# yynil/RWKVTTS

Measured on AMD Instinct MI355X. Metric: audio-tokens/sec/GPU (train fwd+bwd) RWKV7-0.4B L=4096; 1->8 GPU scaling, higher is better.
Workload: dtype bf16; 1 GPU; RWKV7-0.4B Spark layout train step (fwd+bwd+AdamW), B=8/GPU L=4096, synthetic text+speech tokens, random init (BASELINE.json configs[1]); global_batch=8, seq_len=4096, parallelism=dp1, grad_allreduce=none

## Files before the change

rwkvtts_amd/backbone.py:

```python
from __future__ import annotations

import json
import math
import os
from dataclasses import asdict, dataclass, field
from typing import List, Optional

import torch
import torch.nn as nn
import torch.nn.functional as F

from . import fused, ops

HEAD_SIZE = 64


@dataclass
class RWKV7Config:
    hidden_size: int = 1024
    num_hidden_layers: int = 24
    head_dim: int = 64
    vocab_size: int = 8193
    decay_low_rank_dim: int = 64
    a_low_rank_dim: int = 64
# ... 269 lines not shown
            mus, w1s, acts, names = self.lora_branches()
            xr, xk, xv, hs = fused.mix_lora(x, mask, self.x_r, self.x_k, self.x_v, mus, w1s, acts)
            return self.forward_mixed((xr, None, xk, xv, None, None), x, mask, v_first, state, seq_start, resid, dict(zip(names, hs)))
        mixed = fused.token_shift_mix6(x, x_prev, self.x_r, self.x_w, self.x_k, self.x_v,
                                       self.x_a, self.x_g, mask, self._stacked_mix(x.dtype))
        return self.forward_mixed(mixed, x, mask, v_first, state, seq_start, resid)

    def lora_branches(self):
        loras = [self.w_lora, self.a_lora] + ([self.v_lora] if self.layer_idx != 0 else []) + [self.g_lora]
        mus = [self.x_w, self.x_a] + ([self.x_v] if self.layer_idx != 0 else []) + [self.x_g]
        names = ("w", "a") + (("v",) if self.layer_idx != 0 else ()) + ("g",)
        return mus, [l.lora[0].weight for l in loras], [l.activation for l in loras], names

    def mix_params(self):
        return (self.x_r, self.x_w, self.x_k, self.x_v, self.x_a, self.x_g)

    def forward_mixed(self, mixed, x, mask, v_first, state: Optional[LayerState] = None, seq_start=None, resid=None, hid=None,
                      diff_state=False, packed: Optional["_PackedState"] = None):
        xr, xw, xk, xv, xa, xg = mixed
        B, T, D = xr.shape
        H, N = self.num_heads, self.head_dim
        r = self.r_proj(xr)
        k = self.k_proj(xk)
        v_lo = None
        if hid is not None:
            v = self.v_proj(xv)
            w_pre = self.w_lora.lora[2](hid["w"])
            a_pre = self.a_lora.lora[2](hid["a"])
            g = self.g_lora.lora[2](hid["g"])
            v_pre = None if self.layer_idx == 0 else self.v_lora.lora[2](hid["v"])
        else:
            if (self.layer_idx != 0 and DUAL_LINEAR_XV and self.v_proj.bias is None
                    and fused.dual_linear_supported(xv, self.v_proj.weight, self.v_lora.lora[0].weight)):
                v, v_lo = fused.dual_linear(xv, self.v_proj.weight, self.v_lora.lora[0].weight)
            else:
                v = self.v_proj(xv)
            w_pre = self.w_lora(xw)
            a_pre = self.a_lora(xa)
            g = self.g_lora(xg)
            if self.layer_idx == 0:
                v_pre = None
            else:
                v_pre = self.v_lora.forward_from_hidden(v_lo) if v_lo is not None else self.v_lora(xv)
        if self.layer_idx == 0:
            if mask is not None:
                v = v * mask
            v_first = v
        if mask is not None:
            r = r * mask

        def core():
            y, vf_next = fused.tmix_core(r, w_pre, k, v, a_pre, g, v_pre, v_first, self.k_k, self.k_a, self.g_norm.weight,
                                         self.g_norm.bias, self.r_k, mask, H, self.g_norm.eps, self.layer_idx == 0, seq_start)
            if resid is not None and self.o_proj.bias is None:
                x1 = fused.linear_add(y, self.o_proj.weight, resid)
                if x1 is not None:
                    return (x1, True), (v_first if vf_next is None else vf_next)
            return self.o_proj(y), (v_first if vf_next is None else vf_next)

        if hid is not None:
            return core()
        if seq_start is not None or (state is None and torch.is_grad_enabled() and (r.requires_grad or w_pre.requires_grad)
                                     and FUSED_TMIX_CORE):
            return core()
        w, k2, v2, a_in, b_in = fused.tmix_prepare(w_pre, k, v, a_pre, v_pre, v_first, self.k_k, self.k_a, mask,
                                                   H, self.layer_idx == 0)
        if state is None:
            if torch.is_grad_enabled() and (r.requires_grad or w.requires_grad):
                y = ops.RUN_CUDA_RWKV7g(r, w, k2, v2, a_in, b_in)
            else:
                y = ops.wkv7_forward_nograd(r, w, k2, v2, a_in, b_in)
        elif packed is not None:
            w = packed.identity_w(w)
            y, hT = ops.wkv7_state_chunked_seq(state.att_kv, r.contiguous(), w, k2, v2, a_in, b_in, packed.seq_off, packed.nseq)
            _store(state, "att_kv", hT, diff_state)
            _store_last(state, "att_x_prev", x, packed, diff_state)
        elif diff_state:
            y, hT = ops.wkv7_state_chunked(state.att_kv, r.contiguous(), w, k2, v2, a_in, b_in)
            _store(state, "att_kv", hT, True)
            _store(state, "att_x_prev", _last_token(x, mask), True)
        else:
            y = ops.RWKV7_BATCH_OP(state.att_kv, r.contiguous(), w, k2, v2, a_in, b_in)
            _store(state, "att_x_prev", _last_token(x, mask), False)
        y = fused.tmix_post(y, r, k2, v2, g, self.g_norm.weight, self.g_norm.bias, self.r_k, H, self.g_norm.eps)
        return self.o_proj(y), v_first


class RWKV7FeedForward(nn.Module):

    def __init__(self, cfg: RWKV7Config, layer_idx: int):
        super().__init__()
        self.x_k = nn.Parameter(torch.zeros(cfg.hidden_size))
        self.key = Linear(cfg.hidden_size, cfg.intermediate_size, bias=False)
        self.value = Linear(cfg.intermediate_size, cfg.hidden_size, bias=False)

    def forward(self, x, mask, state: Optional[LayerState] = None, diff_state=False, packed: Optional["_PackedState"] = None):
        if packed is not None:
            kx = packed.carry((fused.token_shift_mix1(x, None, self.x_k, mask),), x, state.ffn_x_prev, (self.x_k,))[0]
            _store_last(state, "ffn_x_prev", x, packed, diff_state)
            return self.forward_mixed(kx)
        kx = fused.token_shift_mix1(x, None if state is None else state.ffn_x_prev, self.x_k, mask)
        if state is not None:
            _store(state, "ffn_x_prev", _last_token(x, mask), diff_state)
        return self.forward_mixed(kx)

    def forward_mixed(self, kx):
        if self.key.bias is None and self.value.bias is None:
            out = fused.channel_mix(kx, self.key.weight, self.value.weight)
            if out is not None:
                return out
        s = fused.key_relu_sq(kx, self.key.weight) if self.key.bias is None else None
        if s is None:
            h = self.key(kx)
            if self.value.bias is None:
                out = fused.relu_sq_value(h, self.value.weight)
                if out is not None:
                    return out
            s = fused.relu_sq(h)
        return self.value(s)


class RWKV7Block(nn.Module):
    def __init__(self, cfg: RWKV7Config, layer_idx: int):
        super().__init__()
        self.layer_idx = layer_idx
        D = cfg.hidden_size
        if layer_idx == 0:
            self.pre_norm = nn.LayerNorm(D, eps=cfg.norm_eps, bias=cfg.norm_bias)
        self.attn_norm = nn.LayerNorm(D, eps=cfg.norm_eps, bias=cfg.norm_bias)
        self.attn = RWKV7Attention(cfg, layer_idx)
        self.ffn_norm = nn.LayerNorm(D, eps=cfg.norm_eps, bias=cfg.norm_bias)
        self.ffn = RWKV7FeedForward(cfg, layer_idx)

    def forward(self, x, delta, mask, v_first, state: Optional[LayerState] = None, seq_start=None, diff_state=False,
                packed: Optional["_PackedState"] = None):
        if self.layer_idx == 0:
            if delta is not None:
                x = x + delta
                delta = None
            x = fused.layer_norm(x, self.pre_norm)
        if diff_state or packed is not None:
            if delta is None:
                h = fused.layer_norm(x, self.attn_norm)
            else:
                x, h = fused.add_layer_norm(x, delta, self.attn_norm)
            att, v_first = self.attn(h, mask, v_first, state, diff_state=diff_state, packed=packed)
            x, h = fused.add_layer_norm(x, att, self.ffn_norm)
            return x, self.ffn(h, mask, state, diff_state=diff_state, packed=packed), v_first
        one_pass = fused.add_ln_mix_supported(x, state)
        if one_pass and (FUSED_ADD_LN_MIX6 or FUSED_ADD_LN_MIX6_FWD):
            x, mixed = fused.add_layer_norm_mix(x, delta, self.attn_norm, mask, self.attn.mix_params(), fwd_only=not FUSED_ADD_LN_MIX6)
            att, v_first = self.attn.forward_mixed(mixed, None, mask, v_first, None, seq_start,
                                                   resid=x if FUSED_ADD_LN_MIX1 else None)
        elif (one_pass and FUSED_TMIX_CORE and fused.FUSED_ADD_LN_MIX_LORA_FWD and x.requires_grad
              and fused.mix_lora_supported(x, state, seq_start, self.attn.lora_branches()[1])):
            a = self.attn
            mus, w1s, acts, names = a.lora_branches()
            x, xr, xk, xv, hs = fused.add_layer_norm_mix_lora(x, delta, self.attn_norm, mask, a.x_r, a.x_k, a.x_v, mus, w1s, acts)
            att, v_first = a.forward_mixed((xr, None, xk, xv, None, None), None, mask, v_first, None, seq_start,
                                           x if FUSED_ADD_LN_MIX1 else None, dict(zip(names, hs)))
        else:
            if delta is None:
                h = fused.layer_norm(x, self.attn_norm)
            else:
                x, h = fused.add_layer_norm(x, delta, self.attn_norm)
            att, v_first = self.attn(h, mask, v_first, state, seq_start, resid=x if (one_pass and FUSED_ADD_LN_MIX1) else None)
        if one_pass and FUSED_ADD_LN_MIX1:
            if isinstance(att, tuple):
                x, (kx,) = fused.add_layer_norm_mix(att[0], None, self.ffn_norm, mask, (self.ffn.x_k,))
            else:
                x, (kx,) = fused.add_layer_norm_mix(x, att, self.ffn_norm, mask, (self.ffn.x_k,))
            return x, self.ffn.forward_mixed(kx), v_first
        x, h = fused.add_layer_norm(x, att, self.ffn_norm)
        return x, self.ffn(h, mask, state), v_first


class ModelOutput(dict):

    def __getattr__(self, k):
        try:
            return self[k]
        except KeyError as e:
            raise AttributeError(k) from e

    def __getitem__(self, k):
        if isinstance(k, int):
            return [v for v in self.values() if v is not None][k]
        return super().__getitem__(k)


class RWKV7Model(nn.Module):

    def __init__(self, cfg: RWKV7Config):
        super().__init__()
        self.config = cfg
        self.embeddings = nn.Embedding(cfg.vocab_size, cfg.hidden_size)
        self.layers = nn.ModuleList([RWKV7Block(cfg, i) for i in range(cfg.num_hidden_layers)])
        self.norm = nn.LayerNorm(cfg.hidden_size, eps=cfg.norm_eps, bias=cfg.norm_bias)
        self.gradient_checkpointing = False

    def forward(self, input_ids=None, attention_mask=None, inputs_embeds=None, past_key_values: Optional[Cache] = None,
                use_cache: Optional[bool] = None, cu_seqlens=None, attention_mask_all_ones: Optional[bool] = None, cache_rows=None,
                **kwargs):
        if (input_ids is None) == (inputs_embeds is None):
            raise ValueError("You must specify exactly one of input_ids or inputs_embeds")
        x = self.embeddings(input_ids) if inputs_embeds is None else inputs_embeds
        if cache_rows is not None:
            return self._forward_packed_rows(x, cu_seqlens, past_key_values, cache_rows)
        if cu_seqlens is not None:
            if past_key_values is not None and len(past_key_values) > 0:
                return self._forward_packed_state(x, cu_seqlens, past_key_values)
            return self._forward_packed(x, cu_seqlens)
        B, T, D = x.shape
        if not x.is_cuda:
            raise RuntimeError("RWKV7Model runs on the HIP device only (no CPU path); move the model and inputs to cuda")
        mask = None
        if attention_mask is not None:
            known = attention_mask_all_ones if attention_mask_all_ones is not None else getattr(attention_mask, "_rwkv7_all_ones", None)
            if known is not None and os.environ.get("RWKV7_CHECK_MASK_HINT") == "1":
                assert bool(attention_mask[:, -T:].all()) == bool(known), \
                    "attention mask hint (mark_all_ones / attention_mask_all_ones) contradicts the mask: marked before an in-place edit?"
            if not (known if known is not None else bool(attention_mask[:, -T:].all())):
                mask = attention_mask[:, -T:].to(x.dtype).unsqueeze(-1)
        if use_cache and past_key_values is None:
            past_key_values = Cache.zeros(self.config, B, x.device, x.dtype)
        stateful = past_key_values is not None and len(past_key_values) > 0
        diff_state = stateful and self._differentiable_state(past_key_values, x)
        pad = 0
        gran = ops.CHUNK_T if x.dtype == torch.bfloat16 else ops.CHUNK_LEN
        if not stateful and T % gran != 0:
            pad = gran - T % gran
            x = torch.cat([x.new_zeros(B, pad, D), x], 1)
            m = torch.ones(B, T, 1, dtype=x.dtype, device=x.device) if mask is None else mask
            mask = torch.cat([m.new_zeros(B, pad, 1), m], 1)
        x = self._run_layers(x, mask, past_key_values if stateful else None, diff_state=diff_state)
        if pad:
            x = x[:, pad:]
        if stateful:
            past_key_values.seen_tokens += T
        return ModelOutput(last_hidden_state=x, past_key_values=past_key_values if stateful else None)


    @staticmethod
    def _differentiable_state(cache: Cache, x) -> bool:
        if not torch.is_grad_enabled() or not cache.requires_grad:
            return False
        if x.dtype != torch.bfloat16:
            raise ValueError(f"training through a differentiable cache needs a bf16 model (the chunked backward is bf16 only), got {x.dtype}")
        return True

    def _run_layers(self, x, mask, cache: Optional[Cache], seq_start=None, diff_state=False, packed=None):
        v_first = delta = None
        for i, layer in enumerate(self.layers):
            if self.gradient_checkpointing and self.training and cache is None:
                x, delta, v_first = torch.utils.checkpoint.checkpoint(layer, x, delta, mask, v_first, None, seq_start,
                                                                      use_reentrant=False)
            else:
                x, delta, v_first = layer(x, delta, mask, v_first, None if cache is None else cache[i], seq_start,
                                          diff_state=diff_state, packed=packed)
        return fused.add_layer_norm(x, delta, self.norm)[1] if delta is not None else fused.layer_norm(x, self.norm)

    def _run_packed_aligned(self, x, cu_seqlens, t_al):
        dest, seq_off = _packed_layout(cu_seqlens, x.shape[1], t_al)
        rows = ops.RowMap(dest, t_al, x.device)
        out = self._run_layers(rows.to_aligned(x), rows.keep.to(x.dtype), None, seq_off.to(x.device, non_blocking=True))
        return ModelOutput(last_hidden_state=rows.to_packed(out), past_key_values=None)

    def _forward_packed_state(self, x, cu_seqlens, cache: Cache):
        n_rows = cache[0].att_kv.shape[0]
        cu = [int(c) for c in cu_seqlens.tolist()]
        N = len(cu) - 1
        if n_rows != N:
            raise ValueError(f"cu_seqlens holds {N} sequences but the cache has batch size {n_rows}: a packed row with a cache needs "
                             "one cache row per sequence")
        if x.dtype != torch.bfloat16:
            raise ValueError(f"cu_seqlens with a cache needs a bf16 model (the stateful packed scan is bf16 only), got {x.dtype}")
        if x.shape[0] != 1 or not x.is_cuda:
            raise ValueError("cu_seqlens expects a packed [1, total, D] row on the HIP device")
        total = x.shape[1]
        if any(b < a for a, b in zip(cu[:-1], cu[1:])) or cu[0] < 0 or cu[-1] > total:
            raise ValueError(f"cu_seqlens must be non-decreasing within [0, {total}], got {cu}")
        diff = self._differentiable_state(cache, x)
        lay = ops.packed_state_layout([b - a for a, b in zip(cu[:-1], cu[1:])], torch.is_grad_enabled(), align=_row_align)
        cache.seen_tokens += cu[-1] - cu[0]
        if lay.t_al == 0:
            return ModelOutput(last_hidden_state=x.new_zeros(x.shape), past_key_values=cache)
        dest = torch.full((total,), -1, dtype=torch.int32)
        dest[cu[0]:cu[-1]] = lay.dest
        rows = ops.RowMap(dest, lay.t_al, x.device)
        packed = _PackedState(lay, rows.keep, x.device)
        out = self._run_layers(rows.to_aligned(x), rows.keep.to(x.dtype), cache, diff_state=diff, packed=packed)
        return ModelOutput(last_hidden_state=rows.to_packed(out), past_key_values=cache)

    def _forward_packed_rows(self, x, cu_seqlens, cache: Cache, cache_rows):
        if cu_seqlens is None or cache is None or len(cache) == 0:
            raise ValueError("cache_rows needs cu_seqlens and past_key_values")
        if cache.requires_grad:
            raise ValueError("cache_rows updates the cache in place: a differentiable cache is not supported")
        rows = [int(r) for r in torch.as_tensor(cache_rows).reshape(-1).tolist()]
        n_rows, N = cache[0].att_kv.shape[0], cu_seqlens.numel() - 1
        if len(rows) != N:
            raise ValueError(f"cache_rows names {len(rows)} rows for {N} sequences")
        if len(set(rows)) != N or any(not 0 <= r < n_rows for r in rows):
            raise ValueError(f"cache_rows must be {N} distinct rows in [0, {n_rows}), got {rows}")
        idx = torch.tensor(rows, dtype=torch.int64).to(cache[0].att_kv.device, non_blocking=True)
        sub = Cache([LayerState(s.att_x_prev.index_select(0, idx), s.att_kv.index_select(0, idx), s.ffn_x_prev.index_select(0, idx))
                     for s in cache.states], cache.seen_tokens)
        out = self._forward_packed_state(x, cu_seqlens, sub)
# ... 114 lines not shown
```

rwkvtts_amd/csrc/ln_row.h:

```cpp
#pragma once
#include <type_traits>

#include "../../include/rwkv7_hip.h"
#include "wkv7_common.h"

namespace rwkv7 {

constexpr int kEwMaxThreads = 512;

typedef __bf16 pkbf2_t __attribute__((ext_vector_type(2)));
typedef float pkf2_t __attribute__((ext_vector_type(2)));
__device__ __forceinline__ uint32_t pk_bf16(float a, float b) {
    const pkf2_t v = {a, b};
    return __builtin_bit_cast(uint32_t, __builtin_convertvector(v, pkbf2_t));
}

template <typename T>
struct V8;
template <>
struct V8<bf16_t> {
    static __device__ __forceinline__ void ld(const bf16_t *p, float (&f)[8]) {
        const uint4 r = *reinterpret_cast<const uint4 *>(p);
        f[0] = __uint_as_float(r.x << 16); f[1] = __uint_as_float(r.x & 0xffff0000u);
        f[2] = __uint_as_float(r.y << 16); f[3] = __uint_as_float(r.y & 0xffff0000u);
        f[4] = __uint_as_float(r.z << 16); f[5] = __uint_as_float(r.z & 0xffff0000u);
        f[6] = __uint_as_float(r.w << 16); f[7] = __uint_as_float(r.w & 0xffff0000u);
    }
    static __device__ __forceinline__ void st(bf16_t *p, const float (&f)[8]) {
        uint4 r;
        r.x = pk_bf16(f[0], f[1]);
        r.y = pk_bf16(f[2], f[3]);
        r.z = pk_bf16(f[4], f[5]);
        r.w = pk_bf16(f[6], f[7]);
        *reinterpret_cast<uint4 *>(p) = r;
    }
    static __device__ __forceinline__ float ld1(const bf16_t *p) { return bf2f(p->x); }
};
template <>
struct V8<float> {
    static __device__ __forceinline__ void ld(const float *p, float (&f)[8]) {
        const float4 a = *reinterpret_cast<const float4 *>(p), b = *reinterpret_cast<const float4 *>(p + 4);
        f[0] = a.x; f[1] = a.y; f[2] = a.z; f[3] = a.w; f[4] = b.x; f[5] = b.y; f[6] = b.z; f[7] = b.w;
    }
    static __device__ __forceinline__ void st(float *p, const float (&f)[8]) {
        *reinterpret_cast<float4 *>(p) = make_float4(f[0], f[1], f[2], f[3]);
        *reinterpret_cast<float4 *>(p + 4) = make_float4(f[4], f[5], f[6], f[7]);
    }
    static __device__ __forceinline__ float ld1(const float *p) { return *p; }
};

template <typename T>
struct Raw8;
template <>
struct Raw8<bf16_t> {
    uint4 r;
    __device__ __forceinline__ void load(const bf16_t *p) { r = *reinterpret_cast<const uint4 *>(p); }
    __device__ __forceinline__ void get(float (&f)[8]) const {
        f[0] = __uint_as_float(r.x << 16); f[1] = __uint_as_float(r.x & 0xffff0000u);
        f[2] = __uint_as_float(r.y << 16); f[3] = __uint_as_float(r.y & 0xffff0000u);
        f[4] = __uint_as_float(r.z << 16); f[5] = __uint_as_float(r.z & 0xffff0000u);
        f[6] = __uint_as_float(r.w << 16); f[7] = __uint_as_float(r.w & 0xffff0000u);
    }
};
template <>
struct Raw8<float> {
    float4 a, b;
    __device__ __forceinline__ void load(const float *p) {
        a = *reinterpret_cast<const float4 *>(p);
        b = *reinterpret_cast<const float4 *>(p + 4);
    }
    __device__ __forceinline__ void get(float (&f)[8]) const {
        f[0] = a.x; f[1] = a.y; f[2] = a.z; f[3] = a.w; f[4] = b.x; f[5] = b.y; f[6] = b.z; f[7] = b.w;
    }
};

template <typename T>
__device__ __forceinline__ float round_to(float v);
template <>
__device__ __forceinline__ float round_to<bf16_t>(float v) { return __uint_as_float(pk_bf16(v, v) & 0xffff0000u); }
template <>
__device__ __forceinline__ float round_to<float>(float v) { return v; }

__device__ __forceinline__ float add_pinned(float a, float b) {
    float r;
    asm("v_add_f32 %0, %1, %2" : "=v"(r) : "v"(a), "v"(b));
    return r;
}
__device__ __forceinline__ float sum_slots(const float *red, int ngroups) {
    float t = 0.f;
    for (int i = 0; i < ngroups; i += 4) {
        const float4 v = *reinterpret_cast<const float4 *>(red + i);
        t = add_pinned(add_pinned(add_pinned(add_pinned(t, v.x), v.y), v.z), v.w);
    }
    return t;
}
template <int ROWS>
__device__ __forceinline__ void red_init(float (*red)[kEwMaxThreads / 8]) {
    for (int i = threadIdx.x; i < ROWS * (kEwMaxThreads / 8); i += blockDim.x) (&red[0][0])[i] = 0.f;
    __syncthreads();
}

__device__ __forceinline__ void block_sum2(float &a, float &b, float (*red)[kEwMaxThreads / 8], int ph, int ngroups) {
    a = sum8(a);
    b = sum8(b);
    if ((threadIdx.x & 7) == 0) {
        red[ph][threadIdx.x >> 3] = a;
        red[ph + 1][threadIdx.x >> 3] = b;
    }
    __syncthreads();
    const float ta = sum_slots(red[ph], ngroups), tb = sum_slots(red[ph + 1], ngroups);
    a = ta;
    b = tb;
}

template <typename T>
struct RowPre {
    Raw8<T> xv, bv;
    float m;
};

template <typename T>
__device__ __forceinline__ void add_ln_row(const RowPre<T> &f, long o, bool has_branch, bool has_mask, bool write, T *x_out, T *h_out,
                                           const float (&gm)[8], const float (&bt)[8], float inv_d, float eps, int ng,
                                           float (*red)[kEwMaxThreads / 8], int &ph, float &mu, float &rs, float (&hm)[8]) {
    float v[8];
    f.xv.get(v);
    if (has_branch) {
        float b[8];
        f.bv.get(b);
#pragma unroll
        for (int j = 0; j < 8; j++) v[j] = round_to<T>(v[j] + b[j]);
        if (write) V8<T>::st(x_out + o, v);
    }
    float s = 0.f, dummy = 0.f;
#pragma unroll
    for (int j = 0; j < 8; j++) s += v[j];
    block_sum2(s, dummy, red, ph, ng);
    ph ^= 2;
    mu = s * inv_d;
    float q = 0.f;
    dummy = 0.f;
#pragma unroll
    for (int j = 0; j < 8; j++) {
        v[j] -= mu;
        q = fmaf(v[j], v[j], q);
    }
    block_sum2(q, dummy, red, ph, ng);
    ph ^= 2;
    rs = rsqrtf(q * inv_d + eps);
    const float m = has_mask ? f.m : 1.f;
#pragma unroll
    for (int j = 0; j < 8; j++) hm[j] = round_to<T>(fmaf(v[j] * rs, gm[j], bt[j]));
    if (write && h_out) V8<T>::st(h_out + o, hm);
#pragma unroll
    for (int j = 0; j < 8; j++) hm[j] *= m;
}

inline bool row_width_ok(int D) { return D > 0 && D % 64 == 0 && D <= kEwMaxThreads * 8; }

template <typename... P, typename... A>
int launch_rows(void (*kernel)(P...), int nblocks, int D, hipStream_t st, A... args) {
    (void)hipGetLastError();
    hipLaunchKernelGGL(kernel, dim3(nblocks), dim3(D / 8), 0, st, args...);
    return (int)hipGetLastError();
}

template <int... NS, typename F>
int for_nmix(int nmix, F launch) {
    int rc = RWKV7_ESHAPE;
    (void)((nmix == NS && ((rc = launch(std::integral_constant<int, NS>{})), true)) || ...);
    return rc;
}

}
```

rwkvtts_amd/fused.py:

```python
import ctypes
import os

import torch

from . import _lib

_FWD_BLOCKS = 32768
_MIX_FWD_BLOCKS = 2048
_BWD_BLOCKS = 1024
_MIX_BWD_ROWS = 4
_MIX_BWD_BLOCKS = 1024


def _sfx(t):
    if not t.is_cuda:
        raise NotImplementedError("fused RWKV-7 stages run on the HIP device only (no CPU path)")
    if t.dtype == torch.bfloat16:
        return "bf16"
    if t.dtype == torch.float32:
        return "f32"
    raise TypeError(f"bf16 or fp32 expected, got {t.dtype}")


def _c(t):
# ... 52 lines not shown
    nmix = params.shape[0]
    gs = [torch.zeros_like(x) if g is None else _c(g) for g in gs]
    nb = _grid(B * T, _MIX_BWD_ROWS, _MIX_BWD_BLOCKS)
    dx = torch.empty_like(x)
    part = torch.empty(nb, nmix, D, dtype=torch.float32, device=x.device)
    _call("mix_bwd", x, B, T, D, nmix, _lib.ptr_array(gs), x, xp, mask, params, dx, part, nb, _MIX_BWD_ROWS)
    return dx, part, gs


class _Mix(torch.autograd.Function):

    @staticmethod
    def forward(ctx, x, x_prev, mask, params):
        x, params = _c(x), _c(params)
        xp = None if x_prev is None else _c(x_prev.to(x.dtype))
        out = _mix_fwd(x, xp, mask, params)
        ctx.save_for_backward(x, xp, mask, params)
        ctx.xp_dtype = None if x_prev is None else x_prev.dtype
        return tuple(out[i] for i in range(params.shape[0]))

    @staticmethod
    def backward(ctx, *gs):
        x, xp, mask, params = ctx.saved_tensors
        dx, part, gs = _mix_bwd(gs, x, xp, mask, params)
        dxp = None
        if ctx.needs_input_grad[1]:
            dxp = (params.float().unsqueeze(1) * torch.stack([g[:, 0, :] for g in gs]).float()).sum(0).to(ctx.xp_dtype)
        return dx, dxp, None, _colsum(part, params.dtype)


FUSED_MIX_LORA = os.environ.get("RWKV7_FUSED_MIX_LORA", "1") == "1"
FUSED_MIX_LORA_HITS = [0]
WGRAD_SLABS_WCAT = 32


def _wcat_grads(dx, dG, wcat, x):
    D = x.shape[-1]
    dG2 = _c(dG).view(-1, dG.shape[-1])
    dx.view(-1, D).addmm_(dG2, wcat)
    return wgrad_splitk(dG2, x.view(-1, D), slabs=WGRAD_SLABS_WCAT)


class _MixLora(torch.autograd.Function):

    @staticmethod
    def forward(ctx, x, mask, params, wcat):
        B, T, D = x.shape
        x, params, wcat = _c(x), _c(params), _c(wcat)
        out = _mix_fwd(x, None, mask, params)
        G = torch.mm(x.view(-1, D), wcat.t())
        ctx.save_for_backward(x, mask, params, wcat)
        FUSED_MIX_LORA_HITS[0] += 1
        return (*[out[i] for i in range(params.shape[0])], G.view(B, T, -1))

    @staticmethod
    def backward(ctx, *gs):
        x, mask, params, wcat = ctx.saved_tensors
        nmix = params.shape[0]
        dx, part, _ = _mix_bwd(gs[:nmix], x, None, mask, params)
        dwcat = None if gs[nmix] is None else _wcat_grads(dx, gs[nmix], wcat, x)
        return dx, None, _colsum(part, params.dtype), dwcat


def mix_lora_supported(x, state, seq_start, w1s=None, mask=None):
    if not (FUSED_MIX_LORA and state is None and (seq_start is None or mask is not None) and x.is_cuda and x.dtype == torch.bfloat16 and torch.is_grad_enabled()
            and x.requires_grad and x.dim() == 3 and x.shape[0] * x.shape[1] >= WGRAD_MIN_ROWS and x.shape[-1] % 8 == 0):
        return False
    if w1s is not None:
        w1s = w1s() if callable(w1s) else w1s
        return 0 < len(w1s) <= 4 and all(w.dtype == torch.bfloat16 and w.is_contiguous() and w.dim() == 2 and w.shape[0] % 8 == 0 for w in w1s)
    return True


def _wcat_fwd(w1s, mus):
    ranks = [w.shape[0] for w in w1s]
    D = w1s[0].shape[1]
    wcat = torch.empty(2 * sum(ranks), D, dtype=w1s[0].dtype, device=w1s[0].device)
    _lib.call("rwkv7_mix_lora_wcat_fwd_bf16", wcat, len(w1s), _ints(ranks), _lib.ptr_array(w1s), _lib.ptr_array(mus), D, wcat)
    return wcat


def _wcat_bwd(dwcat, w1s, mus):
    nb = len(w1s)
    D = w1s[0].shape[1]
    dw1 = [torch.empty_like(w) for w in w1s]
    dmu = [torch.empty(D, dtype=w1s[0].dtype, device=w1s[0].device) for _ in range(nb)]
    _lib.call("rwkv7_mix_lora_wcat_bwd_bf16", dwcat, nb, _ints([w.shape[0] for w in w1s]), _lib.ptr_array(w1s), _lib.ptr_array(mus), D,
              dwcat, _lib.ptr_array(dw1), _lib.ptr_array(dmu))
    return dw1, dmu


class _WcatBuild(torch.autograd.Function):

    @staticmethod
    def forward(ctx, nb, *ts):
        w1s, mus = [_c(t) for t in ts[:nb]], [_c(t) for t in ts[nb:]]
        ctx.save_for_backward(*w1s, *mus)
        ctx.nb = nb
        ctx.mu_shapes = [t.shape for t in ts[nb:]]
        return _wcat_fwd(w1s, mus)

    @staticmethod
    def backward(ctx, dwcat):
        ts = ctx.saved_tensors
        dw1, dmu = _wcat_bwd(_c(dwcat), ts[:ctx.nb], ts[ctx.nb:])
        return (None, *dw1, *[g.view(sh) for g, sh in zip(dmu, ctx.mu_shapes)])


_ACT_CODE = {None: 0, "tanh": 1, "sigmoid": 2}


def _combine_bwd(das, outs, mask, ranks, acts, shape):
    B, T = outs[0].shape[:2]
    das = [torch.zeros_like(o) if g is None else _c(g) for g, o in zip(das, outs)]
    dG = torch.empty(shape, dtype=outs[0].dtype, device=outs[0].device)
    _lib.call("rwkv7_mix_lora_combine_bwd_bf16", dG, len(ranks), _ints(ranks), _ints(acts), B * T, T, mask, _lib.ptr_array(outs),
              _lib.ptr_array(das), dG)
    return dG


class _CombineAct(torch.autograd.Function):

    @staticmethod
    def forward(ctx, G, mask, ranks, acts):
        B, T, R2 = G.shape
        G = _c(G)
        outs = [torch.empty(B, T, r, dtype=G.dtype, device=G.device) for r in ranks]
        _lib.call("rwkv7_mix_lora_combine_fwd_bf16", G, len(ranks), _ints(ranks), _ints(acts), B * T, T, G, mask, _lib.ptr_array(outs))
        ctx.save_for_backward(mask, *outs)
        ctx.ranks, ctx.acts, ctx.shape = ranks, acts, (B, T, R2)
        return tuple(outs)

    @staticmethod
    def backward(ctx, *das):
        mask, *outs = ctx.saved_tensors
        return _combine_bwd(das, outs, mask, ctx.ranks, ctx.acts, ctx.shape), None, None, None


LORA_DOWN_DIRECT = os.environ.get("RWKV7_LORA_DOWN_DIRECT", "1") == "1"
LORA_DOWN_DIRECT_HITS = [0]


def lora_down_direct_supported(x, w1s):
    B, T, D = x.shape
    ranks = [w.shape[0] for w in w1s]
    if not (LORA_DOWN_DIRECT and (B * T) % 128 == 0 and D % 128 == 0 and D <= 4096 and all(r % 32 == 0 for r in ranks)):
        return False
    tiles = [b for b, r in enumerate(ranks) for _ in range(r // 32)]
    ok = lambda h: 1 <= len(h) <= 5 and len(set(h)) <= 2
    lds = 2 * (3 * 129 * 72 + 2 * len(tiles) * 2048 + len(ranks) * D)
    return 2 <= len(tiles) <= 10 and lds <= 160 * 1024 and any(ok(tiles[:c]) and ok(tiles[c:]) for c in range(1, len(tiles)))


class _MixLoraDirect(torch.autograd.Function):

    @staticmethod
    def forward(ctx, x, mask, params, nb, acts, *ts):
        B, T, D = x.shape
        x, params = _c(x), _c(params)
        w1s, mus = [_c(t) for t in ts[:nb]], [_c(t.reshape(-1)) for t in ts[nb:]]
        out = _mix_fwd(x, None, mask, params)
        ranks = [w.shape[0] for w in w1s]
        cr = _ints(ranks)
        packed = torch.empty(sum(ranks), D, dtype=x.dtype, device=x.device)
        hs = [torch.empty(B, T, r, dtype=x.dtype, device=x.device) for r in ranks]
        _lib.call("rwkv7_lora_down_pack_bf16", x, nb, cr, _lib.ptr_array(w1s), D, packed)
        _lib.call("rwkv7_lora_down_fwd_bf16", x, nb, cr, _ints(acts), B * T, T, D, x, mask, _lib.ptr_array(mus), packed, _lib.ptr_array(hs))
        ctx.save_for_backward(x, mask, params, *w1s, *mus, *hs)
        ctx.nb, ctx.acts, ctx.mu_shapes = nb, acts, [t.shape for t in ts[nb:]]
        LORA_DOWN_DIRECT_HITS[0] += 1
        FUSED_MIX_LORA_HITS[0] += 1
        return (*[out[i] for i in range(params.shape[0])], *hs)

    @staticmethod
    def backward(ctx, *gs):
        nb = ctx.nb
        x, mask, params, *rest = ctx.saved_tensors
        w1s, mus, hs = rest[:nb], rest[nb:2 * nb], rest[2 * nb:]
        nmix = params.shape[0]
        ranks = [w.shape[0] for w in w1s]
        dG = _combine_bwd(gs[nmix:], hs, mask, ranks, ctx.acts, (x.shape[0] * x.shape[1], 2 * sum(ranks)))
        dx, part, _ = _mix_bwd(gs[:nmix], x, None, mask, params)
        dwcat = _c(_wcat_grads(dx, dG, _wcat_fwd(w1s, mus), x))
        dw1, dmu = _wcat_bwd(dwcat, w1s, mus)
        return (dx, None, _colsum(part, params.dtype), None, None, *dw1, *[g.view(sh) for g, sh in zip(dmu, ctx.mu_shapes)])


def mix_lora(x, mask, x_r, x_k, x_v, mus, w1s, acts):
    B, T, D = x.shape
    params = torch.cat([p.reshape(1, D) for p in (x_r, x_k, x_v)], 0).to(x.dtype)
    mr = _mask_rows(mask, x)
    if lora_down_direct_supported(x, w1s):
        outs = _MixLoraDirect.apply(x, mr, params, len(w1s), tuple(_ACT_CODE[a] for a in acts), *w1s, *mus)
        return outs[0], outs[1], outs[2], list(outs[3:])
    wcat = _WcatBuild.apply(len(w1s), *w1s, *mus)
    xr, xk, xv, G = _MixLora.apply(x, mr, params, wcat)
    hs = _CombineAct.apply(G, mr, tuple(w.shape[0] for w in w1s), tuple(_ACT_CODE[a] for a in acts))
    return xr, xk, xv, list(hs)


def token_shift_mix6(x, x_prev, x_r, x_w, x_k, x_v, x_a, x_g, mask=None, stacked=None):
    D = x.shape[-1]
    params = stacked if stacked is not None else torch.cat([p.reshape(1, D) for p in (x_r, x_w, x_k, x_v, x_a, x_g)], 0).to(x.dtype)
    return _Mix.apply(x, x_prev, _mask_rows(mask, x), params)


def token_shift_mix1(x, x_prev, x_k, mask=None):
    return _Mix.apply(x, x_prev, _mask_rows(mask, x), x_k.reshape(1, -1).to(x.dtype))[0]


class _ReluSq(torch.autograd.Function):
    @staticmethod
    def forward(ctx, x):
        x = _c(x)
        y = torch.empty_like(x)
        _call("relusq_fwd", x, x.numel(), x, y)
        ctx.save_for_backward(x)
        return y

    @staticmethod
    def backward(ctx, dy):
        (x,) = ctx.saved_tensors
        dy = _c(dy)
        dx = torch.empty_like(x)
        _call("relusq_bwd", x, x.numel(), x, dy, dx)
        return dx


def relu_sq(x):
    return _ReluSq.apply(x)


FUSED_KEY_RELUSQ = os.environ.get("RWKV7_FUSED_KEY_RELUSQ", "0") == "1"
FUSED_KEY_RELUSQ_HITS = [0]


def key_relusq_eligible(x, weight):
    M = x.numel() // x.shape[-1]
    return (FUSED_KEY_RELUSQ and x.is_cuda and x.dtype == torch.bfloat16 and weight.dtype == torch.bfloat16 and M % 256 == 0
            and weight.shape[0] % 256 == 0 and weight.shape[1] % 1024 == 0)


class _KeyReluSq(torch.autograd.Function):
    @staticmethod
    def forward(ctx, x, weight):
        x2 = _c(x).view(-1, x.shape[-1])
        w = _c(weight)
        M, K = x2.shape
        N = w.shape[0]
        s = torch.empty(M, N, dtype=x.dtype, device=x.device)
        _lib.call("rwkv7_gemm_nt_bf16", x, M, N, K, x2, w, s, 1)
        FUSED_KEY_RELUSQ_HITS[0] += 1
        ctx.save_for_backward(x, weight, s)
        ctx.wparam = weight
        return s.view(*x.shape[:-1], N)

    @staticmethod
    def backward(ctx, ds):
        x, weight, s = ctx.saved_tensors
        ds2 = _c(ds).view(-1, ds.shape[-1])
        dk = torch.empty_like(s)
        _call("relusq_bwd_s", s, s.numel(), s, ds2, dk)
        x2 = _c(x).view(-1, x.shape[-1])
        dx = _dgrad(dk, weight).view(x.shape) if ctx.needs_input_grad[0] else None
        dw = None
        if ctx.needs_input_grad[1]:
            dw = _wgrad(dk, x2, ctx.wparam)
        return dx, dw


FUSED_RELUSQ_VALUE_BWD = os.environ.get("RWKV7_FUSED_RELUSQ_VALUE_BWD", "0") == "1"


def relusq_value_eligible(h, weight):
    M = h.numel() // h.shape[-1]
    return (FUSED_RELUSQ_VALUE_BWD and h.is_cuda and h.dtype == torch.bfloat16 and weight.dtype == torch.bfloat16 and M % 256 == 0
            and weight.shape[1] % 256 == 0 and weight.shape[0] % 1024 == 0 and torch.is_grad_enabled())


class _ReluSqValue(torch.autograd.Function):

    @staticmethod
    def forward(ctx, h, weight):
        h2 = _c(h).view(-1, h.shape[-1])
        s = torch.empty_like(h2)
        _call("relusq_fwd", h2, h2.numel(), h2, s)
        out = torch.nn.functional.linear(s, weight)
        ctx.save_for_backward(h2, s, weight)
        ctx.wparam = weight
        ctx.shape = h.shape
        return out.view(*h.shape[:-1], weight.shape[0])

    @staticmethod
    def backward(ctx, dout):
        h2, s, weight = ctx.saved_tensors
        d2 = _c(dout).view(-1, dout.shape[-1])
        M, F = h2.shape
        D = weight.shape[0]
        dh = None
        if ctx.needs_input_grad[0]:
            wt = weight.detach().t().contiguous()
            dh = torch.empty_like(h2)
            _lib.call("rwkv7_gemm_nt_relusq_bwd_bf16", h2, M, F, D, d2, wt, h2, dh)
            dh = dh.view(ctx.shape)
        dw = _wgrad(d2, s, ctx.wparam) if ctx.needs_input_grad[1] else None
        return dh, dw


FUSED_CMIX = os.environ.get("RWKV7_FUSED_CMIX", "1") == "1"
FUSED_CMIX_HITS = [0]
DGRAD_NT = os.environ.get("RWKV7_DGRAD_NT", "1") == "1"
DGRAD_NT_MIN_N = int(os.environ.get("RWKV7_DGRAD_NT_MIN_N", "2048"))
DGRAD_NT_HITS = [0]


def _dgrad(dy2, weight):
    N, K = weight.shape
    if (DGRAD_NT and dy2.is_cuda and dy2.dtype == torch.bfloat16 and weight.dtype == torch.bfloat16 and dy2.shape[0] >= WGRAD_MIN_ROWS
            and N % 64 == 0 and K % 64 == 0 and N >= DGRAD_NT_MIN_N and K >= 256 and weight.is_contiguous() and dy2.is_contiguous()):
        wt = torch.empty(K, N, dtype=weight.dtype, device=weight.device)
        _lib.call("rwkv7_transpose_bf16", dy2, N, K, weight, wt)
        DGRAD_NT_HITS[0] += 1
        return torch.mm(dy2, wt.t())
    return torch.mm(dy2, weight)


TRANSPOSE_KERNEL = True


def cmix_eligible(x, wk, wv):
    M = x.numel() // x.shape[-1]
    return (FUSED_CMIX and x.is_cuda and x.dtype == torch.bfloat16 and wk.dtype == torch.bfloat16 and wv.dtype == torch.bfloat16
            and M % 256 == 0 and wk.shape[0] % 256 == 0 and wk.shape[1] % 1024 == 0 and wv.shape[0] == wk.shape[1] and wv.shape[1] == wk.shape[0])


class _ChannelMix(torch.autograd.Function):

    @staticmethod
# ... 421 lines not shown
        ctx.params = (wa, wb)
        ctx.set_materialize_grads(False)
        return torch.nn.functional.linear(x, wa), torch.nn.functional.linear(x, wb)

    @staticmethod
    def backward(ctx, dya, dyb):
        x, wa, wb = ctx.saved_tensors
        K = x.shape[-1]
        x2 = _c(x).view(-1, K)
        da2 = None if dya is None else _c(dya).view(-1, wa.shape[0])
        db2 = None if dyb is None else _c(dyb).view(-1, wb.shape[0])
        dx = None
        if ctx.needs_input_grad[0]:
            if da2 is not None and db2 is not None:
                dx = _dgrad(da2, wa)
                dx.addmm_(db2, wb)
            elif da2 is not None:
                dx = _dgrad(da2, wa)
            elif db2 is not None:
                dx = torch.mm(db2, wb)
            dx = None if dx is None else dx.view(x.shape)
        grads = []
        for i, (d2, w) in enumerate(((da2, wa), (db2, wb))):
            g = None
            if d2 is not None and ctx.needs_input_grad[1 + i]:
                g = _wgrad(d2, x2, ctx.params[i])
            grads.append(g)
        return dx, grads[0], grads[1]


def dual_linear_supported(x, wa, wb):
    return (x.is_cuda and x.dtype == torch.bfloat16 and torch.is_grad_enabled() and wa.requires_grad and wb.requires_grad
            and x.numel() // x.shape[-1] >= WGRAD_MIN_ROWS)


def dual_linear(x, wa, wb):
    return _DualLinear.apply(x, wa, wb)


GEMV_MAX_ROWS = 32


def linear(x, weight, bias=None):
    rows = x.numel() // x.shape[-1]
    if (GEMV_MAX_ROWS and x.is_cuda and x.dtype == torch.bfloat16 and rows <= GEMV_MAX_ROWS and x.shape[-1] % 64 == 0
            and not (torch.is_grad_enabled() and (x.requires_grad or weight.requires_grad)) and weight.dtype == torch.bfloat16):
        K, N = x.shape[-1], weight.shape[0]
        x2, w2 = _c(x).view(rows, K), _c(weight)
        b2 = None if bias is None else _c(bias.to(torch.bfloat16))
        y = torch.empty(rows, N, dtype=torch.bfloat16, device=x.device)
        _lib.call("rwkv7_gemv32_bf16", x, rows, N, K, x2, w2, b2, y)
        return y.view(*x.shape[:-1], N)
    if (x.is_cuda and x.dtype == torch.bfloat16 and torch.is_grad_enabled() and weight.requires_grad
            and x.numel() // x.shape[-1] >= WGRAD_MIN_ROWS):
        return _Linear.apply(x, weight, bias)
    return torch.nn.functional.linear(x, weight, bias)


FUSED_OPROJ_ADD = os.environ.get("RWKV7_FUSED_OPROJ_ADD", "1") == "1"


def linear_add_eligible(y, weight, resid):
    M = y.numel() // y.shape[-1]
    return (FUSED_OPROJ_ADD and y.is_cuda and y.dtype == torch.bfloat16 and weight.dtype == torch.bfloat16 and resid.dtype == torch.bfloat16
            and M % 256 == 0 and weight.shape[0] % 256 == 0 and weight.shape[1] % 1024 == 0 and resid.shape == (*y.shape[:-1], weight.shape[0]))


class _LinearAdd(torch.autograd.Function):

    @staticmethod
    def forward(ctx, y, weight, resid):
        y2 = _c(y).view(-1, y.shape[-1])
        w = _c(weight)
        r2 = _c(resid).view(-1, resid.shape[-1])
        M, K = y2.shape
        N = w.shape[0]
        out = torch.empty(M, N, dtype=y.dtype, device=y.device)
        _lib.call("rwkv7_gemm_nt_add_bf16", y, M, N, K, y2, w, r2, out)
        ctx.save_for_backward(y2, weight)
        ctx.wparam = weight
        ctx.yshape = y.shape
        return out.view(resid.shape)

    @staticmethod
    def backward(ctx, d1):
        y2, weight = ctx.saved_tensors
        d2 = _c(d1).view(-1, d1.shape[-1])
        dy = _dgrad(d2, weight).view(ctx.yshape) if ctx.needs_input_grad[0] else None
        dw = _wgrad(d2, y2, ctx.wparam) if ctx.needs_input_grad[1] else None
        return dy, dw, (d1 if ctx.needs_input_grad[2] else None)


def linear_add(y, weight, resid):
    if linear_add_eligible(y, weight, resid):
        return _LinearAdd.apply(y, weight, resid)
    return None


def _ln_params(gamma, beta, dtype):
    return _c(gamma.to(dtype)), (None if beta is None else _c(beta.to(dtype)))


def _add_ln_bwd(dh, d_x1, xs, mean, rstd, gamma):
    D = xs.shape[-1]
    rows = xs.numel() // D
    nb = min(rows, _BWD_BLOCKS)
    dx = torch.empty_like(xs)
    part = torch.empty(nb, 2, D, dtype=torch.float32, device=xs.device)
    _call("add_ln_bwd", xs, rows, D, _c(dh), _c_opt(d_x1), xs, mean, rstd, gamma, dx, part, nb)
    dp = _colsum(part, xs.dtype)
    return dx, dp[0], dp[1]


class _AddLN(torch.autograd.Function):

    @staticmethod
    def forward(ctx, x, branch, gamma, beta, eps):
        D = x.shape[-1]
        x = _c(x)
        rows = x.numel() // D
        gamma_c, beta_c = _ln_params(gamma, beta, x.dtype)
        h = torch.empty_like(x)
        mean = torch.empty(rows, dtype=torch.float32, device=x.device)
        rstd = torch.empty_like(mean)
        if branch is not None:
            branch = _c(branch)
            x1 = torch.empty_like(x)
        else:
            x1 = None
        _call("add_ln_fwd", x, rows, D, x, branch, gamma_c, beta_c, eps, x1, h, mean, rstd, min(rows, _FWD_BLOCKS))
        ctx.has_branch, ctx.has_beta = branch is not None, beta is not None
        ctx.save_for_backward(x1 if branch is not None else x, mean, rstd, gamma_c)
        if branch is None:
            return h
        return x1, h

    @staticmethod
    def backward(ctx, *grads):
        xs, mean, rstd, gamma = ctx.saved_tensors
        if ctx.has_branch:
            d_x1, dh = grads
        else:
            d_x1, dh = None, grads[0]
        if dh is None:
            dx = d_x1
            return dx, (dx if ctx.has_branch else None), None, None, None
        dx, dgamma, dbeta = _add_ln_bwd(dh, d_x1, xs, mean, rstd, gamma)
        return dx, (dx if ctx.has_branch else None), dgamma, (dbeta if ctx.has_beta else None), None


_ADD_LN_MIX_RUN = 4
_ADD_LN_MIX_BLOCKS = 8192
_ADD_LN_MIX_BWD_BLOCKS = 2048


def _add_ln_mix_fwd(x, branch, gamma, beta, eps, mask, params, store_h):
    B, T, D = x.shape
    nmix = params.shape[0]
    gamma_c, beta_c = _ln_params(gamma, beta, x.dtype)
    out = torch.empty(nmix, B, T, D, dtype=x.dtype, device=x.device)
    h = torch.empty_like(x) if store_h else None
    mean = torch.empty(B * T, dtype=torch.float32, device=x.device)
    rstd = torch.empty_like(mean)
    x1 = None if branch is None else torch.empty_like(x)
    nb = _grid(B * T, _ADD_LN_MIX_RUN, _ADD_LN_MIX_BLOCKS)
    _call("add_ln_mix_fwd_h" if store_h else "add_ln_mix_fwd", x, B, T, D, nmix, x, _c_opt(branch), gamma_c, beta_c, eps, mask, params, x1,
          out, *((h,) if store_h else ()), mean, rstd, nb, _ADD_LN_MIX_RUN)
    return (x if branch is None else x1), out, h, mean, rstd, gamma_c, beta_c


class _AddLNMix(torch.autograd.Function):

    @staticmethod
    def forward(ctx, x, branch, gamma, beta, eps, mask, params):
        x, params = _c(x), _c(params)
        x1, out, _, mean, rstd, gamma_c, beta_c = _add_ln_mix_fwd(x, branch, gamma, beta, eps, mask, params, store_h=False)
        ctx.has_branch, ctx.has_beta = branch is not None, beta is not None
        ctx.save_for_backward(x1, mean, rstd, gamma_c, beta_c, mask, params)
        return (x1,) + tuple(out[i] for i in range(params.shape[0]))

    @staticmethod
    def backward(ctx, d_x1, *gs):
        xs, mean, rstd, gamma, beta, mask, params = ctx.saved_tensors
        B, T, D = xs.shape
        nmix = params.shape[0]
        gs = [torch.zeros_like(xs) if g is None else _c(g) for g in gs]
        nb = _grid(B * T, _ADD_LN_MIX_RUN, _ADD_LN_MIX_BWD_BLOCKS)
        dx = torch.empty_like(xs)
        part = torch.empty(nb, nmix + 2, D, dtype=torch.float32, device=xs.device)
        _call("mix_add_ln_bwd", xs, B, T, D, nmix, _lib.ptr_array(gs), _c_opt(d_x1), xs, mean, rstd, gamma, beta, mask, params, dx, part, nb,
              _ADD_LN_MIX_RUN)
        dp = _colsum(part, xs.dtype) if params.dtype == xs.dtype else part.sum(0)
        return (dx, (dx if ctx.has_branch else None), dp[nmix].to(xs.dtype), (dp[nmix + 1].to(xs.dtype) if ctx.has_beta else None),
                None, None, dp[:nmix].to(params.dtype))


FUSED_ADD_LN_MIX_LORA_FWD = os.environ.get("RWKV7_FUSED_ADD_LN_MIX_LORA_FWD", "0") == "1"


class _AddLNMixFwd(torch.autograd.Function):

    @staticmethod
    def forward(ctx, x, branch, gamma, beta, eps, mask, params, wcat):
        B, T, D = x.shape
        x, params, wcat = _c(x), _c(params), _c_opt(wcat)
        x1, out, h, mean, rstd, gamma_c, _ = _add_ln_mix_fwd(x, branch, gamma, beta, eps, mask, params, store_h=True)
        ctx.has_branch, ctx.has_beta = branch is not None, beta is not None
        ctx.save_for_backward(x1, h, mean, rstd, gamma_c, mask, params, wcat)
        outs = (x1, *[out[i] for i in range(params.shape[0])])
        if wcat is None:
            return outs
        FUSED_MIX_LORA_HITS[0] += 1
        return (*outs, torch.mm(h.view(-1, D), wcat.t()).view(B, T, -1))

    @staticmethod
    def backward(ctx, d_x1, *gs):
        xs, h, mean, rstd, gamma, mask, params, wcat = ctx.saved_tensors
        nmix = params.shape[0]
        dh, part_m, _ = _mix_bwd(gs[:nmix], h, None, mask, params)
        dwcat = None
        if wcat is not None and gs[nmix] is not None:
            dwcat = _wcat_grads(dh, gs[nmix], wcat, h)
        dx, dgamma, dbeta = _add_ln_bwd(dh, d_x1, xs, mean, rstd, gamma)
        return (dx, (dx if ctx.has_branch else None), dgamma, (dbeta if ctx.has_beta else None), None, None,
                _colsum(part_m, params.dtype), dwcat)


def add_layer_norm_mix_lora(x, branch, norm, mask, x_r, x_k, x_v, mus, w1s, acts):
    D = x.shape[-1]
    params = torch.cat([p.reshape(1, D) for p in (x_r, x_k, x_v)], 0).to(x.dtype)
    wcat = _WcatBuild.apply(len(w1s), *w1s, *mus)
    mr = _mask_rows(mask, x)
    x1, xr, xk, xv, G = _AddLNMixFwd.apply(x, branch, norm.weight, norm.bias, norm.eps, mr, params, wcat)
    hs = _CombineAct.apply(G, mr, tuple(w.shape[0] for w in w1s), tuple(_ACT_CODE[a] for a in acts))
    return x1, xr, xk, xv, list(hs)


def add_ln_mix_supported(x, state):
    return x.is_cuda and state is None and x.dim() == 3 and x.dtype in (torch.bfloat16, torch.float32) and torch.is_grad_enabled()


def add_layer_norm_mix(x, branch, norm, mask, mix_params, fwd_only=False):
    D = x.shape[-1]
    params = torch.cat([p.reshape(1, D) for p in mix_params], 0).to(x.dtype) if len(mix_params) > 1 else mix_params[0].reshape(1, D).to(x.dtype)
    args = (x, branch, norm.weight, norm.bias, norm.eps, _mask_rows(mask, x), params)
    res = _AddLNMixFwd.apply(*args, None) if (fwd_only and len(mix_params) > 1) else _AddLNMix.apply(*args)
    return res[0], res[1:]


def layer_norm(x, norm):
    return _AddLN.apply(x, None, norm.weight, norm.bias, norm.eps)


def add_layer_norm(x, branch, norm):
    return _AddLN.apply(x, branch, norm.weight, norm.bias, norm.eps)
```

Before: 278,300 tokens/s.

## Enable fused add+LayerNorm+mix with direct LoRA-down path by default

Turns on the fused add+LayerNorm+token-mix+LoRA-down forward path by default. It also adds a new autograd function that feeds the stored normalized activations into the direct LoRA-down kernel instead of a concatenated-weight matmul plus a combine/activation step. The aim is to remove separate LayerNorm, mix and LoRA projection launches and intermediate tensors in each time-mix block. The LayerNorm row reduction now uses a single-value block sum instead of a paired sum with a dummy, and the fused forward with stored h uses longer row runs and fewer blocks. The risks are a changed numerical path and extra saved activations (h) for backward.

```diff
diff --git a/rwkvtts_amd/backbone.py b/rwkvtts_amd/backbone.py
--- a/rwkvtts_amd/backbone.py
+++ b/rwkvtts_amd/backbone.py
@@ -445,8 +445,8 @@
             x, mixed = fused.add_layer_norm_mix(x, delta, self.attn_norm, mask, self.attn.mix_params(), fwd_only=not FUSED_ADD_LN_MIX6)
             att, v_first = self.attn.forward_mixed(mixed, None, mask, v_first, None, seq_start,
                                                    resid=x if FUSED_ADD_LN_MIX1 else None)
-        elif (one_pass and FUSED_TMIX_CORE and fused.FUSED_ADD_LN_MIX_LORA_FWD and x.requires_grad
-              and fused.mix_lora_supported(x, state, seq_start, self.attn.lora_branches()[1])):
+        elif (one_pass and FUSED_TMIX_CORE and fused.add_ln_mix_lora_eligible(x)
+              and fused.mix_lora_supported(x, state, seq_start, lambda: self.attn.lora_branches()[1], mask)):
             a = self.attn
             mus, w1s, acts, names = a.lora_branches()
             x, xr, xk, xv, hs = fused.add_layer_norm_mix_lora(x, delta, self.attn_norm, mask, a.x_r, a.x_k, a.x_v, mus, w1s, acts)
diff --git a/rwkvtts_amd/csrc/ln_row.h b/rwkvtts_amd/csrc/ln_row.h
--- a/rwkvtts_amd/csrc/ln_row.h
+++ b/rwkvtts_amd/csrc/ln_row.h
@@ -113,6 +113,13 @@
     b = tb;
 }
 
+__device__ __forceinline__ void block_sum1(float &a, float (*red)[kEwMaxThreads / 8], int ph, int ngroups) {
+    a = sum8(a);
+    if ((threadIdx.x & 7) == 0) red[ph][threadIdx.x >> 3] = a;
+    __syncthreads();
+    a = sum_slots(red[ph], ngroups);
+}
+
 template <typename T>
 struct RowPre {
     Raw8<T> xv, bv;
@@ -132,20 +139,19 @@
         for (int j = 0; j < 8; j++) v[j] = round_to<T>(v[j] + b[j]);
         if (write) V8<T>::st(x_out + o, v);
     }
-    float s = 0.f, dummy = 0.f;
+    float s = 0.f;
 #pragma unroll
     for (int j = 0; j < 8; j++) s += v[j];
-    block_sum2(s, dummy, red, ph, ng);
+    block_sum1(s, red, ph, ng);
     ph ^= 2;
     mu = s * inv_d;
     float q = 0.f;
-    dummy = 0.f;
 #pragma unroll
     for (int j = 0; j < 8; j++) {
         v[j] -= mu;
         q = fmaf(v[j], v[j], q);
     }
-    block_sum2(q, dummy, red, ph, ng);
+    block_sum1(q, red, ph, ng);
     ph ^= 2;
     rs = rsqrtf(q * inv_d + eps);
     const float m = has_mask ? f.m : 1.f;
diff --git a/rwkvtts_amd/fused.py b/rwkvtts_amd/fused.py
--- a/rwkvtts_amd/fused.py
+++ b/rwkvtts_amd/fused.py
@@ -228,38 +228,48 @@
     return 2 <= len(tiles) <= 10 and lds <= 160 * 1024 and any(ok(tiles[:c]) and ok(tiles[c:]) for c in range(1, len(tiles)))
 
 
+def _lora_down_direct_fwd(x, mask, w1s, mus, acts):
+    B, T, D = x.shape
+    nb = len(w1s)
+    ranks = [w.shape[0] for w in w1s]
+    cr = _ints(ranks)
+    packed = torch.empty(sum(ranks), D, dtype=x.dtype, device=x.device)
+    hs = [torch.empty(B, T, r, dtype=x.dtype, device=x.device) for r in ranks]
+    _lib.call("rwkv7_lora_down_pack_bf16", x, nb, cr, _lib.ptr_array(w1s), D, packed)
+    _lib.call("rwkv7_lora_down_fwd_bf16", x, nb, cr, _ints(acts), B * T, T, D, x, mask, _lib.ptr_array(mus), packed, _lib.ptr_array(hs))
+    LORA_DOWN_DIRECT_HITS[0] += 1
+    FUSED_MIX_LORA_HITS[0] += 1
+    return hs
+
+
+def _mix_lora_direct_bwd(gs, acts, x, mask, params, w1s, mus, hs):
+    nmix = params.shape[0]
+    ranks = [w.shape[0] for w in w1s]
+    dG = _combine_bwd(gs[nmix:], hs, mask, ranks, acts, (x.shape[0] * x.shape[1], 2 * sum(ranks)))
+    dx, part, _ = _mix_bwd(gs[:nmix], x, None, mask, params)
+    dwcat = _c(_wcat_grads(dx, dG, _wcat_fwd(w1s, mus), x))
+    dw1, dmu = _wcat_bwd(dwcat, w1s, mus)
+    return dx, _colsum(part, params.dtype), dw1, dmu
+
+
 class _MixLoraDirect(torch.autograd.Function):
 
     @staticmethod
     def forward(ctx, x, mask, params, nb, acts, *ts):
-        B, T, D = x.shape
         x, params = _c(x), _c(params)
         w1s, mus = [_c(t) for t in ts[:nb]], [_c(t.reshape(-1)) for t in ts[nb:]]
         out = _mix_fwd(x, None, mask, params)
-        ranks = [w.shape[0] for w in w1s]
-        cr = _ints(ranks)
-        packed = torch.empty(sum(ranks), D, dtype=x.dtype, device=x.device)
-        hs = [torch.empty(B, T, r, dtype=x.dtype, device=x.device) for r in ranks]
-        _lib.call("rwkv7_lora_down_pack_bf16", x, nb, cr, _lib.ptr_array(w1s), D, packed)
-        _lib.call("rwkv7_lora_down_fwd_bf16", x, nb, cr, _ints(acts), B * T, T, D, x, mask, _lib.ptr_array(mus), packed, _lib.ptr_array(hs))
+        hs = _lora_down_direct_fwd(x, mask, w1s, mus, acts)
         ctx.save_for_backward(x, mask, params, *w1s, *mus, *hs)
         ctx.nb, ctx.acts, ctx.mu_shapes = nb, acts, [t.shape for t in ts[nb:]]
-        LORA_DOWN_DIRECT_HITS[0] += 1
-        FUSED_MIX_LORA_HITS[0] += 1
         return (*[out[i] for i in range(params.shape[0])], *hs)
 
     @staticmethod
     def backward(ctx, *gs):
         nb = ctx.nb
         x, mask, params, *rest = ctx.saved_tensors
-        w1s, mus, hs = rest[:nb], rest[nb:2 * nb], rest[2 * nb:]
-        nmix = params.shape[0]
-        ranks = [w.shape[0] for w in w1s]
-        dG = _combine_bwd(gs[nmix:], hs, mask, ranks, ctx.acts, (x.shape[0] * x.shape[1], 2 * sum(ranks)))
-        dx, part, _ = _mix_bwd(gs[:nmix], x, None, mask, params)
-        dwcat = _c(_wcat_grads(dx, dG, _wcat_fwd(w1s, mus), x))
-        dw1, dmu = _wcat_bwd(dwcat, w1s, mus)
-        return (dx, None, _colsum(part, params.dtype), None, None, *dw1, *[g.view(sh) for g, sh in zip(dmu, ctx.mu_shapes)])
+        dx, dparams, dw1, dmu = _mix_lora_direct_bwd(gs, ctx.acts, x, mask, params, rest[:nb], rest[nb:2 * nb], rest[2 * nb:])
+        return (dx, None, dparams, None, None, *dw1, *[g.view(sh) for g, sh in zip(dmu, ctx.mu_shapes)])
 
 
 def mix_lora(x, mask, x_r, x_k, x_v, mus, w1s, acts):
@@ -987,6 +997,7 @@
 _ADD_LN_MIX_RUN = 4
 _ADD_LN_MIX_BLOCKS = 8192
 _ADD_LN_MIX_BWD_BLOCKS = 2048
+_ADD_LN_MIX_H_RUN_X, _ADD_LN_MIX_H_BLOCKS_DIV = 2, 4
 
 
 def _add_ln_mix_fwd(x, branch, gamma, beta, eps, mask, params, store_h):
@@ -998,9 +1009,10 @@
     mean = torch.empty(B * T, dtype=torch.float32, device=x.device)
     rstd = torch.empty_like(mean)
     x1 = None if branch is None else torch.empty_like(x)
-    nb = _grid(B * T, _ADD_LN_MIX_RUN, _ADD_LN_MIX_BLOCKS)
+    run = _ADD_LN_MIX_RUN * (_ADD_LN_MIX_H_RUN_X if store_h else 1)
+    nb = _grid(B * T, run, max(1, _ADD_LN_MIX_BLOCKS // (_ADD_LN_MIX_H_BLOCKS_DIV if store_h else 1)))
     _call("add_ln_mix_fwd_h" if store_h else "add_ln_mix_fwd", x, B, T, D, nmix, x, _c_opt(branch), gamma_c, beta_c, eps, mask, params, x1,
-          out, *((h,) if store_h else ()), mean, rstd, nb, _ADD_LN_MIX_RUN)
+          out, *((h,) if store_h else ()), mean, rstd, nb, run)
     return (x if branch is None else x1), out, h, mean, rstd, gamma_c, beta_c
 
 
@@ -1030,7 +1042,8 @@
                 None, None, dp[:nmix].to(params.dtype))
 
 
-FUSED_ADD_LN_MIX_LORA_FWD = os.environ.get("RWKV7_FUSED_ADD_LN_MIX_LORA_FWD", "0") == "1"
+FUSED_ADD_LN_MIX_LORA_FWD = os.environ.get("RWKV7_FUSED_ADD_LN_MIX_LORA_FWD", "1") == "1"
+ADD_LN_MIX_LORA_HITS = [0]
 
 
 class _AddLNMixFwd(torch.autograd.Function):
@@ -1061,14 +1074,46 @@
                 _colsum(part_m, params.dtype), dwcat)
 
 
+class _AddLNMixLoraDirect(torch.autograd.Function):
+
+    @staticmethod
+    def forward(ctx, x, branch, gamma, beta, eps, mask, params, nb, acts, *ts):
+        x, params = _c(x), _c(params)
+        w1s, mus = [_c(t) for t in ts[:nb]], [_c(t.reshape(-1)) for t in ts[nb:]]
+        x1, out, h, mean, rstd, gamma_c, _ = _add_ln_mix_fwd(x, branch, gamma, beta, eps, mask, params, store_h=True)
+        hs = _lora_down_direct_fwd(h, mask, w1s, mus, acts)
+        ctx.has_branch, ctx.has_beta = branch is not None, beta is not None
+        ctx.save_for_backward(x1, h, mean, rstd, gamma_c, mask, params, *w1s, *mus, *hs)
+        ctx.nb, ctx.acts, ctx.mu_shapes = nb, acts, [t.shape for t in ts[nb:]]
+        return ((x1 if ctx.has_branch else None), *[out[i] for i in range(params.shape[0])], *hs)
+
+    @staticmethod
+    def backward(ctx, d_x1, *gs):
+        nb = ctx.nb
+        xs, h, mean, rstd, gamma, mask, params, *rest = ctx.saved_tensors
+        dh, dparams, dw1, dmu = _mix_lora_direct_bwd(gs, ctx.acts, h, mask, params, rest[:nb], rest[nb:2 * nb], rest[2 * nb:])
+        dx, dgamma, dbeta = _add_ln_bwd(dh, d_x1, xs, mean, rstd, gamma)
+        return (dx, (dx if ctx.has_branch else None), dgamma, (dbeta if ctx.has_beta else None), None, None, dparams, None, None,
+                *dw1, *[g.view(sh) for g, sh in zip(dmu, ctx.mu_shapes)])
+
+
+def add_ln_mix_lora_eligible(x):
+    return FUSED_ADD_LN_MIX_LORA_FWD and x.is_cuda and x.dtype == torch.bfloat16 and x.dim() == 3 and x.shape[-1] % 64 == 0
+
+
 def add_layer_norm_mix_lora(x, branch, norm, mask, x_r, x_k, x_v, mus, w1s, acts):
     D = x.shape[-1]
     params = torch.cat([p.reshape(1, D) for p in (x_r, x_k, x_v)], 0).to(x.dtype)
+    mr = _mask_rows(mask, x)
+    ADD_LN_MIX_LORA_HITS[0] += 1
+    if lora_down_direct_supported(x, w1s):
+        x1, xr, xk, xv, *hs = _AddLNMixLoraDirect.apply(x, branch, norm.weight, norm.bias, norm.eps, mr, params, len(w1s),
+                                                        tuple(_ACT_CODE[a] for a in acts), *w1s, *mus)
+        return (x if branch is None else x1), xr, xk, xv, list(hs)
     wcat = _WcatBuild.apply(len(w1s), *w1s, *mus)
-    mr = _mask_rows(mask, x)
     x1, xr, xk, xv, G = _AddLNMixFwd.apply(x, branch, norm.weight, norm.bias, norm.eps, mr, params, wcat)
     hs = _CombineAct.apply(G, mr, tuple(w.shape[0] for w in w1s), tuple(_ACT_CODE[a] for a in acts))
-    return x1, xr, xk, xv, list(hs)
+    return (x if branch is None else x1), xr, xk, xv, list(hs)
 
 
 def add_ln_mix_supported(x, state):
```

Result: no change. 280,200 tokens/s, median of 6 (+0.7%).
